# Edresson/VoiceSplit

Hardware: AMD Instinct MI355X
Metric: utterances/sec (3 s clips, B=64/GPU) fwd+bwd, channels-last bf16 activations / tape, bf16 MFMA, fp32 accumulate / statistics / master weights (higher is better)
Workload: dtype bf16 (conv activations and tape stored as bf16; bf16 MFMA operands in the convs, the LSTM / head contractions and the BPTT, f16 operands in the forward recurrence; fp32 accumulate, BatchNorm statistics, gate arithmetic / cell state, loss head, master weights)

## Files before the change

### include/voicesplit_hip.h

```cpp
#ifndef VOICESPLIT_HIP_H
#define VOICESPLIT_HIP_H

#include <stddef.h>
#include <stdint.h>

#ifdef __cplusplus
extern "C" {
#endif
#if defined(__GNUC__)
#pragma GCC visibility push(default)
#endif

#define VS_ABI_VERSION 11

#define VS_ACT_RELU 0
#define VS_ACT_MISH 1
#define VS_ACT_NONE 2
#define VS_ACT_SIGMOID 3

#define VS_MATH_FP32 0
#define VS_MATH_F16X3 1
#define VS_MATH_BF16 2

#define VS_BN_EVAL 0
// ... 227 lines not shown
  size_t total_bytes;
  size_t z[7];
  size_t a[7];
  size_t z8;
  size_t feat;
  size_t bn_scale, bn_shift, bn_mean, bn_invstd;
  size_t gates;
  size_t cstate;
  size_t lstm_out;
  size_t fc1_out;
  size_t dlogits;
  size_t dfc1;
  size_t dlstm_out;
  size_t dsum;
  size_t dfeat;
  size_t grad0, grad1;
  size_t dvbias, conv_packed[6], pack_tmp, lstm_packed, lstm_packed_t, lstm_state, lstm_bwd_state;
  size_t consts;
  size_t bn_stats, bn_coef, first_acc, colsum_tmp, partials;
  size_t conv_scales;
  size_t gemm_scales;
  size_t lstm_bf16;
  size_t det_turn;
  size_t conv_packed_t[6];
} vs_tape_layout;

int vs_tape_layout_query(const vs_dims* dims, vs_tape_layout* out);
size_t vs_tape_bytes(const vs_dims* dims);

int vs_forward_train(const vs_dims* dims, const vs_params* params, const float* x, const float* dvec,
                     int conv_act, int bn_mode, void* tape, size_t tape_bytes, float* mask, void* stream);

int vs_backward(const vs_dims* dims, const vs_params* params, const float* x, const float* dvec,
                int conv_act, int bn_mode, void* tape, size_t tape_bytes,
                const float* mask, const float* dmask, const vs_grads* grads, void* stream);

int vs_conv64_pack_dgrad(const float* w, float* packed, int KT, int KF, void* stream);
size_t vs_conv64_wgrad_partial_floats(int KT, int KF);
int vs_conv64_wgrad(const float* dz, const float* in, float* partials, float* dw,
                    int B, int T, int F, int KT, int KF, int dil, void* stream);
int vs_conv64_wgrad_f16x3(const float* dz, const float* in, float* partials, float* dw, float* scratch8,
                          int B, int T, int F, int KT, int KF, int dil, void* stream);
int vs_set_wgrad_kernel(int mode);
int vs_set_conv_kernel(int mode);
int vs_set_lstm_kernel(int mode);

enum vs_option {
  VS_OPT_FWD_PROLOGUE = 0,
  VS_OPT_HEAD_LEAF_SIDE = 1,
  VS_OPT_FEAT_ROWS = 2,
  VS_OPT_HEAD_BWD_GEMM = 3,
  VS_OPT_ABLATION = 4,
  VS_OPT_DETERMINISTIC = 5,
  VS_OPT_COUNT = 6
};
int vs_set_option(int option, int value);
int vs_get_option(int option);

int vs_lstm_status(const vs_dims* dims, const void* tape, size_t tape_bytes, const void* workspace, size_t workspace_bytes, void* stream);

int vs_set_backward_overlap(int on);
int vs_bn_act_bwd(const float* da, const float* z, float* dz, int C, long long R, int L, int act, int bn_mode,
                  const float* scale, const float* shift, const float* mean, const float* invstd,
                  float* dgamma, float* dbeta, float* dbias, double* stats, float* coef, void* stream);
int vs_bn_act_bwd_first(const float* da, const float* z, const float* x, float* xpad, int B, int T, int F, int act, int bn_mode,
                        const float* scale, const float* shift, const float* mean, const float* invstd,
                        float* dgamma, float* dbeta, float* dbias, float* dw, double* stats, float* coef, double* acc, void* stream);
int vs_conv_last_dgrad(const float* dz, const float* w, float* din, int B, int T, int F, void* stream);
int vs_conv_last_wgrad_blocks(void);
int vs_conv_last_wgrad(const float* dz, const float* in, float* partials , float* dw,
                       int B, int T, int F, void* stream);
int vs_conv_first_wgrad(const float* dz, const float* x, double* acc, float* dw, int B, int T, int F, void* stream);
int vs_gemm(int layout_a, int layout_w, const float* A, int lda, const float* W, int ldw, float* C, int ldc,
            int M, int N, int K, const float* bias, const float* gate, int ldg, int a_relu, int w_relu, int act,
            int accumulate, int w_shift, int w_group, int splits, float* partials, void* stream);
int vs_gemm_f16x3(int layout_a, int layout_w, const float* A, int lda, const float* W, int ldw, float* C, int ldc,
                  int M, int N, int K, const float* bias, const float* gate, int ldg, int a_relu, int w_relu, int act,
                  int accumulate, float* scratch8, void* stream);
int vs_bilstm_recurrent_train(const float* xg, const float* packed_whh, float* state, float* out,
                              float* gates_save, float* c_save, int B, int T, int H, void* stream);
size_t vs_lstm_packed_t_floats(int H);
size_t vs_lstm_bwd_state_floats(int B, int H);
int vs_lstm_pack_t(const float* w_hh_fwd, const float* w_hh_bwd, float* packed_t, int H, void* stream);
int vs_bilstm_recurrent_bwd(const float* packed_t, float* state, float* gates, const float* c_all,
                            const float* dout, int B, int T, int H, void* stream);
int vs_lstm_pack_t_math(const float* w_hh_fwd, const float* w_hh_bwd, float* packed_t, int H, int math, void* stream);
int vs_bilstm_recurrent_bwd_math(const float* packed_t, float* state, float* gates, const float* c_all,
                                 const float* dout, int B, int T, int H, int math, void* stream);
int vs_sigmoid_bwd(const float* dmask, const float* mask, float* dlogits, long long n, void* stream);
int vs_colsum(const float* x, int ld, int groups, int rows, int N, float* out, int ldo, void* stream);

typedef struct vs_loss_dims {
  int B, T, F;
  int n_fft, hop, win;
  float min_level_db;
  float ref_level_db;
} vs_loss_dims;

size_t vs_sisnr_workspace_bytes(const vs_loss_dims* dims);
int vs_sisnr_loss(const vs_loss_dims* dims, const float* mixed, const float* mask, const float* target,
                  const float* phase, const int* seq_len, void* workspace, size_t workspace_bytes,
                  float* loss, float* dmask, float* est_wav, void* stream);

int vs_powerlaw_loss(const float* mixed, const float* mask, const float* target, long long n, float power,
                     float complex_loss_ratio, double* scratch, float* loss, float* dmask, void* stream);

size_t vs_audio_workspace_bytes(const vs_loss_dims* dims);
// ... 170 lines not shown
```

### voicesplit_amd/_lib.py

```python
import ctypes
import os
from ctypes import POINTER, Structure, c_char_p, c_double, c_float, c_int, c_longlong, c_size_t, c_void_p

_HERE = os.path.dirname(os.path.abspath(__file__))
LIB_PATH = os.path.join(_HERE, "libvoicesplit_hip.so")

ACT_RELU, ACT_MISH, ACT_NONE, ACT_SIGMOID = 0, 1, 2, 3
BN_EVAL, BN_TRAIN = 0, 1
MATH_FP32, MATH_F16X3, MATH_BF16 = 0, 1, 2
PROF_SLOTS = 29
PROF_NAMES = ("cnn1", "cnn2", "cnn3", "cnn4", "cnn5", "cnn6", "cnn7", "cnn8", "lstm_gemm", "lstm_rec", "head",
              "fwd_bn", "bwd_head", "bwd_lstm_rec", "bwd_lstm_gemm", "bwd_bn",
              "wgrad_cnn2", "wgrad_cnn3", "wgrad_cnn4", "wgrad_cnn5", "wgrad_cnn6", "wgrad_cnn7",
              "dgrad_cnn2", "dgrad_cnn3", "dgrad_cnn4", "dgrad_cnn5", "dgrad_cnn6", "dgrad_cnn7", "bwd_edge")
ABI_VERSION = 11
CODEC_DB01, CODEC_DBNORM, CODEC_LOG = 0, 1, 2
PAD_REFLECT, PAD_ZERO = 0, 1


class VsDims(Structure):
    _fields_ = [(n, c_int) for n in ("B", "T", "F", "E", "H", "FC1", "FC2", "math")]


class VsConvLayer(Structure):
# ... 233 lines not shown
    "vs_split_workspace_bytes": (c_size_t, [c_longlong, c_int]),
    "vs_split_point": (c_int, [_P, c_longlong, _P, _P, _P, c_int, _P, _P, _P, c_int, _P, c_size_t, _P]),
    "vs_mix_sequence": (c_int, [_P, c_longlong, _P, c_longlong, _P, c_int, c_int, c_int, _P, _P, _P, _P, _P, _P, _P, _P]),
    "vs_resample_plan": (c_int, [c_int, c_int, POINTER(VsResampleDims)]),
    "vs_resample_out_len": (c_longlong, [POINTER(VsResampleDims), c_longlong]),
    "vs_resample_bank": (c_int, [POINTER(VsResampleDims), _P, _P]),
    "vs_resample": (c_int, [POINTER(VsResampleDims), _P, _P, c_longlong, c_longlong, c_longlong, c_longlong, _P, c_longlong, c_longlong,
                            c_longlong, c_int, _P]),
    "vs_resample_clips": (c_int, [POINTER(VsResampleDims), _P, _P, c_longlong, _P, c_longlong, _P, _P, c_int, _P]),
    "vs_loudness_plan": (c_int, [c_int, POINTER(VsLoudnessDims)]),
    "vs_loudness_workspace_bytes": (c_size_t, [POINTER(VsLoudnessDims), c_longlong, c_int]),
    "vs_loudness": (c_int, [POINTER(VsLoudnessDims), _P, c_longlong, _P, _P, c_int, _P, _P, _P, _P, _P, _P, _P, c_size_t, _P]),
    "vs_scale_clips": (c_int, [_P, c_longlong, _P, _P, _P, c_int, _P]),
    "vs_stoi_plan": (c_int, [POINTER(VsStoiDims)]),
    "vs_stoi_workspace_bytes": (c_size_t, [POINTER(VsStoiDims), c_longlong, c_int]),
    "vs_stoi": (c_int, [POINTER(VsStoiDims), _P, _P, c_longlong, _P, _P, c_int, c_int, _P, _P, _P, _P, _P, _P, c_size_t, _P]),
    "vs_rir_shoebox": (c_int, [_P, _P, c_int, c_int, _P, _P]),
    "vs_fir_rows": (c_int, [_P, c_longlong, _P, _P, _P, _P, c_int, c_int, _P, c_int, c_int, c_int, _P, _P, _P, _P]),
    "vs_row_energy": (c_int, [_P, c_int, c_int, _P, _P]),
    "vs_fir_spectra_bytes": (c_size_t, [c_int, c_int]),
    "vs_fir_spectra": (c_int, [_P, _P, _P, c_int, c_int, _P, c_size_t, _P]),
    "vs_fir_fft_workspace_bytes": (c_size_t, [c_int, c_int, c_int]),
    "vs_fir_rows_fft": (c_int, [_P, c_longlong, _P, _P, _P, c_int, c_int, _P, c_size_t, c_int, c_int, _P, c_size_t, _P, _P, _P]),
}

_lib = None


class VoiceSplitHipError(RuntimeError):
    pass


def load(path: str = None) -> ctypes.CDLL:
    global _lib
    if _lib is not None and path is None:
        return _lib
    path = path or LIB_PATH
    if not os.path.isfile(path):
        raise VoiceSplitHipError(
            f"{path} not found: build it with `python -c 'import __graft_entry__ as g; g.build()'` "
            f"or `make -C voicesplit_amd/csrc`. There is no PyTorch/CPU fallback for this path.")
    lib = ctypes.CDLL(path)
    for name, (restype, argtypes) in SIGNATURES.items():
        fn = getattr(lib, name)
        fn.restype = restype
        fn.argtypes = argtypes
    if lib.vs_abi_version() != ABI_VERSION:
        raise VoiceSplitHipError(f"{path}: ABI version {lib.vs_abi_version()} != {ABI_VERSION}; rebuild")
    _apply_env_options(lib)
    _lib = lib
    return lib


OPTIONS = {"FWD_PROLOGUE": 0, "HEAD_LEAF_SIDE": 1, "FEAT_ROWS": 2, "HEAD_BWD_GEMM": 3, "ABLATION": 4, "DETERMINISTIC": 5}
_ENV_OPTIONS = {
    "VOICESPLIT_FWD_PROLOGUE": ("FWD_PROLOGUE", int),
    "VOICESPLIT_HEAD_LEAF_SIDE": ("HEAD_LEAF_SIDE", int),
    "VOICESPLIT_FEAT_ROWS": ("FEAT_ROWS", int),
    "VOICESPLIT_HEAD_BWD_GEMM": ("HEAD_BWD_GEMM", int),
    "VOICESPLIT_ABLATION": ("ABLATION", int),
    "VOICESPLIT_DETERMINISTIC": ("DETERMINISTIC", int),
}


def _apply_env_options(lib):
    for var, (name, conv) in _ENV_OPTIONS.items():
        v = os.environ.get(var)
        if v is None or v == "":
            continue
        try:
            value = conv(v)
        except ValueError as err:
            raise VoiceSplitHipError(f"{var}={v}: not a value of this switch ({err})") from None
        if lib.vs_set_option(OPTIONS[name], value) != 0:
            msg = lib.vs_last_error()
            raise VoiceSplitHipError(f"{var}={v}: {msg.decode() if msg else 'rejected by vs_set_option'}")


def set_option(name: str, value: int):
    lib = load()
    prev = lib.vs_get_option(OPTIONS[name])
    check(lib.vs_set_option(OPTIONS[name], int(value)), f"vs_set_option({name})")
    return prev


def get_option(name: str) -> int:
    return load().vs_get_option(OPTIONS[name])


def check(rc: int, what: str):
    if rc != 0:
        msg = load().vs_last_error()
        raise VoiceSplitHipError(f"{what} failed (rc={rc}): {msg.decode() if msg else '?'}")
```

### voicesplit_amd/csrc/capi.hip

```cpp
#include <stdarg.h>
#include <stdlib.h>
#include <string.h>

#include "../../include/voicesplit_hip.h"
#include "vs_internal.h"

static thread_local char g_err[512] = "";

void vs_set_error(const char* fmt, ...) {
  va_list ap;
  va_start(ap, fmt);
  vsnprintf(g_err, sizeof(g_err), fmt, ap);
  va_end(ap);
}

int g_vs_options[VS_OPT_COUNT] = { 1,  1,  1,  1,  0,  0};
thread_local unsigned* g_vs_turn = nullptr;

namespace {
struct Prof {
  bool on = false;
  int max_calls = 0;
  int calls[VS_PROF_SLOTS] = {0};
  hipEvent_t* ev = nullptr;
} g_prof;

}

VsProfScope::VsProfScope(int slot, hipStream_t s_) : s(s_), idx(-1) {
  if (!g_prof.on || g_prof.calls[slot] >= g_prof.max_calls) return;
  idx = (g_prof.calls[slot]++ * VS_PROF_SLOTS + slot) * 2;
  (void)hipEventRecord(g_prof.ev[idx], s);
}
VsProfScope::~VsProfScope() { if (idx >= 0) (void)hipEventRecord(g_prof.ev[idx + 1], s); }

extern "C" {

int vs_abi_version(void) { return VS_ABI_VERSION; }

int vs_set_option(int option, int value) {
  VS_REQUIRE(option >= 0 && option < VS_OPT_COUNT, "vs_set_option: unknown option %d", option);
  bool ok = true;
  switch (option) {
    case VS_OPT_FWD_PROLOGUE: case VS_OPT_HEAD_LEAF_SIDE: case VS_OPT_FEAT_ROWS: case VS_OPT_HEAD_BWD_GEMM: case VS_OPT_DETERMINISTIC:
      ok = value == 0 || value == 1; break;
    default: ok = value >= 0; break;
  }
  VS_REQUIRE(ok, "vs_set_option: value %d is outside the range of option %d", value, option);
  g_vs_options[option] = value;
  return 0;
}

int vs_get_option(int option) { return (option >= 0 && option < VS_OPT_COUNT) ? g_vs_options[option] : -1; }

int vs_profile_begin(int max_calls) {
  VS_REQUIRE(!g_prof.on, "profile: already enabled");
  VS_REQUIRE(max_calls > 0 && max_calls <= 4096, "profile: max_calls=%d out of range", max_calls);
  max_calls *= 8;
  const int n = max_calls * VS_PROF_SLOTS * 2;
  g_prof.ev = new hipEvent_t[n];
  for (int i = 0; i < n; ++i) VS_CHECK_HIP(hipEventCreate(&g_prof.ev[i]));
  for (int i = 0; i < VS_PROF_SLOTS; ++i) g_prof.calls[i] = 0;
  g_prof.max_calls = max_calls;
  g_prof.on = true;
  return 0;
}

int vs_profile_end(float* ms_total, int* calls) {
  VS_REQUIRE(g_prof.on, "profile: not enabled");
  g_prof.on = false;
  int rc = 0;
  for (int slot = 0; slot < VS_PROF_SLOTS; ++slot) {
    double tot = 0;
    for (int c = 0; c < g_prof.calls[slot]; ++c) {
      const int idx = (c * VS_PROF_SLOTS + slot) * 2;
      float ms = 0.f;
      hipError_t e = hipEventSynchronize(g_prof.ev[idx + 1]);
      if (e == hipSuccess) e = hipEventElapsedTime(&ms, g_prof.ev[idx], g_prof.ev[idx + 1]);
      if (e != hipSuccess) { vs_set_error("profile: %s", hipGetErrorString(e)); rc = -2; }
      tot += ms;
    }
    if (ms_total) ms_total[slot] = (float)tot;
    if (calls) calls[slot] = g_prof.calls[slot];
  }
  const int n = g_prof.max_calls * VS_PROF_SLOTS * 2;
  for (int i = 0; i < n; ++i) (void)hipEventDestroy(g_prof.ev[i]);
  delete[] g_prof.ev;
  g_prof.ev = nullptr;
  g_prof.max_calls = 0;
  return rc;
}
const char* vs_last_error(void) { return g_err; }

int vs_bn_fold(const float* gamma, const float* beta, const float* mean, const float* var, const float* conv_bias,
               float eps, int C, float* scale, float* shift, void* stream) {
  return vs_bn_fold_impl(gamma, beta, mean, var, conv_bias, eps, C, scale, shift, (hipStream_t)stream);
}
// ... 347 lines not shown
```

### voicesplit_amd/csrc/loss.hip

```cpp
#include <math.h>

#include "../../include/voicesplit_hip.h"
#include "stft_common.h"

namespace {

__global__ __launch_bounds__(256)
void overlap_add_bwd_kernel(const float* __restrict__ dwav, const float* __restrict__ env, float* __restrict__ dframes, VsStftShape s,
                            unsigned* __restrict__ amax = nullptr) {
  const long long n = (long long)s.B * s.T * s.win;
  float mx = 0.f;
  for (long long i = (long long)blockIdx.x * 256 + threadIdx.x; i < n; i += (long long)gridDim.x * 256) {
    const long long m = i / s.win;
    const int j = (int)(i - m * s.win);
    const int b = (int)(m / s.T), t = (int)(m - (long long)b * s.T);
    const int sp = s.hop * t - s.lead + j;
    const float v = (sp >= 0 && sp < s.S) ? dwav[(size_t)b * s.S + sp] / env[sp] : 0.f;
    dframes[i] = v;
    mx = fmaxf(mx, fabsf(v));
  }
  vs_absmax_commit(mx, amax);
}

__global__ __launch_bounds__(256)
void sisnr_moments_kernel(const float* __restrict__ est, const float* __restrict__ src, const int* __restrict__ len,
                          double* __restrict__ mom , VsStftShape s) {
  const int b = blockIdx.y;
  const int L = len ? (len[b] < s.S ? (len[b] > 0 ? len[b] : 0) : s.S) : s.S;
  double a[6] = {0, 0, 0, 0, 0, 0};
  for (int i = blockIdx.x * 256 + threadIdx.x; i < s.S; i += gridDim.x * 256) {
    const double e = est[(size_t)b * s.S + i], r = src[(size_t)b * s.S + i];
    a[0] += r;
    if (i < L) { a[1] += e; a[2] += r; a[3] += e * r; a[4] += e * e; a[5] += r * r; }
  }
  __shared__ double red[4][6];
#pragma unroll
  for (int q = 0; q < 6; ++q) {
#pragma unroll
    for (int o = 32; o > 0; o >>= 1) a[q] += __shfl_down(a[q], o, 64);
  }
  if ((threadIdx.x & 63) == 0) {
#pragma unroll
    for (int q = 0; q < 6; ++q) red[threadIdx.x >> 6][q] = a[q];
  }
  __syncthreads();
  if (threadIdx.x < 6) atomicAdd(&mom[b * 8 + threadIdx.x], (red[0][threadIdx.x] + red[1][threadIdx.x]) + (red[2][threadIdx.x] + red[3][threadIdx.x]));
}

__global__ void sisnr_finalize_kernel(const double* __restrict__ mom, const int* __restrict__ len, float* __restrict__ coef ,
                                      float* __restrict__ loss, VsStftShape s) {
  __shared__ double acc[64];
  const int tid = threadIdx.x;
  double part = 0.0;
  const double eps = 1e-16;
  for (int b = tid; b < s.B; b += 64) {
    const double nlen = len ? (double)len[b] : (double)s.S;
    const int Lm_i = len ? (len[b] < s.S ? (len[b] > 0 ? len[b] : 0) : s.S) : s.S;
    const double Lm = Lm_i;
    const double* m = mom + b * 8;
    const double mu_s = m[0] / nlen, mu_e = m[1] / nlen;
    const double Sze = m[1] - Lm * mu_e, Szs = m[2] - Lm * mu_s;
    const double dot = m[3] - mu_s * m[1] - mu_e * m[2] + Lm * mu_e * mu_s;
    const double Z = m[5] - 2 * mu_s * m[2] + Lm * mu_s * mu_s;
    const double E = m[4] - 2 * mu_e * m[1] + Lm * mu_e * mu_e;
    const double es = Z + eps;
    const double P = dot * dot * Z / (es * es);
    const double c = (es + eps) / (es * es);
    const double N = E - c * dot * dot + eps;
    const double snr = P / N;
    part += 10.0 * log10(snr + eps);
    const double k = 10.0 / (log(10.0) * (snr + eps)) * (-1.0 / s.B);
    const double gs = k * (2 * dot * Z / (es * es) / N + P / (N * N) * 2 * c * dot);
    const double ge = k * (-P / (N * N) * 2);
    const double gsum = gs * Szs + ge * Sze;
    float* o = coef + b * 8;
    o[0] = (float)gs; o[1] = (float)ge; o[2] = (float)(gsum / nlen); o[3] = (float)mu_s; o[4] = (float)mu_e;
    o[5] = (float)Lm_i;
  }
  acc[tid] = part;
  __syncthreads();
  if (tid == 0) {
    double t = 0;
    for (int i = 0; i < 64; ++i) t += acc[i];
    *loss = (float)(20.0 - t / s.B);
  }
}

__global__ __launch_bounds__(256)
void sisnr_grad_kernel(const float* __restrict__ est, const float* __restrict__ src, const float* __restrict__ coef,
                       float* __restrict__ dwav, VsStftShape s) {
  const int b = blockIdx.y;
  const float gs = coef[b * 8], ge = coef[b * 8 + 1], g0 = coef[b * 8 + 2], mu_s = coef[b * 8 + 3], mu_e = coef[b * 8 + 4];
  const int L = (int)coef[b * 8 + 5];
  for (int i = blockIdx.x * 256 + threadIdx.x; i < s.S; i += gridDim.x * 256) {
    float g = 0.f;
    if (i < L) {
      const float zs = src[(size_t)b * s.S + i] - mu_s, ze = est[(size_t)b * s.S + i] - mu_e;
      g = fmaf(gs, zs, fmaf(ge, ze, -g0));
    }
    dwav[(size_t)b * s.S + i] = g;
  }
}

__global__ __launch_bounds__(256)
void reim_to_dmask_kernel(const float* __restrict__ mixed, const float* __restrict__ mask, const float* __restrict__ phase,
                          const float* __restrict__ dreim, float* __restrict__ dmask, VsStftShape s) {
  const long long n = (long long)s.B * s.T * s.F;
  for (long long i = (long long)blockIdx.x * 256 + threadIdx.x; i < n; i += (long long)gridDim.x * 256) {
    const long long m = i / s.F;
    const int f = (int)(i - m * s.F);
    const float x = mixed[i], v = x * mask[i];
    float g = 0.f;
    if (v >= 0.f && v <= 1.f) {
      const float db = (v - 1.f) * (-s.min_level_db) + s.ref_level_db;
      const float mag = expf(db * kLn10Over20);
      float sn, cs;
      sincosf(phase[i], &sn, &cs);
      const float d = dreim[m * s.ldk + f] * expf(cs) + dreim[m * s.ldk + s.F + f] * expf(sn);
      g = x * (-s.min_level_db) * kLn10Over20 * mag * d;
    }
    dmask[i] = g;
  }
}

__global__ __launch_bounds__(256)
void powerlaw_kernel(const float* __restrict__ mixed, const float* __restrict__ mask, const float* __restrict__ target,
                     long long n, float power, float ratio, double* __restrict__ sums, float* __restrict__ dmask) {
  constexpr float kEps = 1e-16f;
  const float inv_n = (float)(1.0 / (double)n);
  double a0 = 0.0, a1 = 0.0;
  for (long long i = (long long)blockIdx.x * 256 + threadIdx.x; i < n; i += (long long)gridDim.x * 256) {
    const float mx = mixed[i];
    const float o = mx * mask[i] + kEps;
    const float t = target[i] + kEps;
    const float po = powf(o, power), pt = powf(t, power);
    const float ds = fabsf(pt) - fabsf(po), dc = pt - po;
    a0 += (double)(ds * ds);
    a1 += (double)(dc * dc);
    if (dmask) {
      const float sgn = po > 0.f ? 1.f : (po < 0.f ? -1.f : 0.f);
      const float dpo = (-2.f * ds * sgn - 2.f * ratio * dc) * inv_n;
      dmask[i] = mx * (power * powf(o, power - 1.f)) * dpo;
    }
  }
#pragma unroll
  for (int off = 32; off > 0; off >>= 1) {
    a0 += __shfl_down(a0, off, 64);
    a1 += __shfl_down(a1, off, 64);
  }
  __shared__ double sh[8];
  const int lane = threadIdx.x & 63, w = threadIdx.x >> 6;
  if (lane == 0) { sh[2 * w] = a0; sh[2 * w + 1] = a1; }
  __syncthreads();
  if (threadIdx.x == 0) {
    atomicAdd(&sums[0], sh[0] + sh[2] + sh[4] + sh[6]);
    atomicAdd(&sums[1], sh[1] + sh[3] + sh[5] + sh[7]);
  }
}

__global__ void powerlaw_finalize_kernel(const double* __restrict__ sums, long long n, float ratio, float* __restrict__ loss) {
  *loss = (float)(sums[0] / (double)n + (double)ratio * (sums[1] / (double)n));
}

}

extern "C" {

size_t vs_sisnr_workspace_bytes(const vs_loss_dims* d) {
  VsStftShape s;
  return vs_stft_make_shape(d, &s) ? 0 : vs_stft_layout(s).total;
}

int vs_sisnr_loss(const vs_loss_dims* d, const float* mixed, const float* mask, const float* target, const float* phase,
                  const int* seq_len, void* ws, size_t ws_bytes, float* loss, float* dmask, float* est_wav, void* stream_) {
  hipStream_t stream = (hipStream_t)stream_;
  VsStftShape s;
  if (int rc = vs_stft_make_shape(d, &s)) return rc;
  const VsStftLayout L = vs_stft_layout(s);
  VS_REQUIRE(mixed && mask && target && phase && loss, "sisnr_loss: NULL argument");
  if (int rc = vs_stft_check_envelope(s)) return rc;
  VS_REQUIRE(ws && (reinterpret_cast<uintptr_t>(ws) & 255) == 0 && ws_bytes >= L.total, "sisnr_loss: workspace too small or misaligned (%zu < %zu)", ws_bytes, L.total);
  const int M = s.B * s.T;
  const long long nspec = (long long)M * s.F;
  float* basis = at<float>(ws, L.basis);
  float* env = at<float>(ws, L.env);
  const bool split = vs_stft_split(s);
  unsigned* amax = at<unsigned>(ws, L.amax);
  float* scales = at<float>(ws, L.scales);
  vs_istft_basis_launch(basis, s, scales + 6, stream);
  vs_istft_envelope_launch(env, s, stream);
  float* reim[2] = {at<float>(ws, L.reim_e), at<float>(ws, L.reim_t)};
  float* frames[2] = {at<float>(ws, L.frames_e), at<float>(ws, L.frames_t)};
  float* wav[2] = {at<float>(ws, L.wav_e), at<float>(ws, L.wav_t)};
  if (split) VS_CHECK_HIP(hipMemsetAsync(amax, 0, (size_t)3 * VS_AMAX_SLOTS * 4, stream));
  const unsigned cap = split ? 2048 : 16384;
  vs_spec_to_reim_launch(mixed, mask, phase, reim[0], s, split ? amax : nullptr, vs_grid_for(nspec, cap), stream);
  vs_spec_to_reim_launch(target, nullptr, phase, reim[1], s, split ? amax + VS_AMAX_SLOTS : nullptr, vs_grid_for(nspec, cap), stream);
  for (int q = 0; q < 2; ++q) {
    if (split) if (int rc = vs_scale_from_absmax_impl(amax + q * VS_AMAX_SLOTS, VS_AMAX_SLOTS, scales + 2 * q, stream)) return rc;
    if (int rc = vs_stft_contract(split, 0, reim[q], s.ldk, basis, s.ldk, frames[q], s.win, M, s.win, s.K, scales + 2 * q, scales + 6, stream)) return rc;
    vs_overlap_add_launch(frames[q], env, wav[q], s, stream);
  }
  if (est_wav) VS_CHECK_HIP(hipMemcpyAsync(est_wav, wav[0], (size_t)s.B * s.S * 4, hipMemcpyDeviceToDevice, stream));
  double* mom = at<double>(ws, L.mom);
  float* coef = at<float>(ws, L.coef);
  VS_CHECK_HIP(hipMemsetAsync(mom, 0, (size_t)s.B * 8 * 8, stream));
  const int gx = vs_opt(VS_OPT_DETERMINISTIC) ? 1 : (s.S + 256 * 16 - 1) / (256 * 16);
  hipLaunchKernelGGL(sisnr_moments_kernel, dim3(gx, s.B), dim3(256), 0, stream, wav[0], wav[1], seq_len, mom, s);
  hipLaunchKernelGGL(sisnr_finalize_kernel, dim3(1), dim3(64), 0, stream, mom, seq_len, coef, loss, s);
  if (dmask) {
    float* dwav = at<float>(ws, L.dwav);
    hipLaunchKernelGGL(sisnr_grad_kernel, dim3(gx, s.B), dim3(256), 0, stream, wav[0], wav[1], coef, dwav, s);
    float* dframes = frames[0];
    hipLaunchKernelGGL(overlap_add_bwd_kernel, dim3(vs_grid_for((long long)M * s.win, cap)), dim3(256), 0, stream, dwav, env, dframes, s,
                       split ? amax + 2 * VS_AMAX_SLOTS : nullptr);
    float* dreim = reim[0];
    if (split) if (int rc = vs_scale_from_absmax_impl(amax + 2 * VS_AMAX_SLOTS, VS_AMAX_SLOTS, scales + 4, stream)) return rc;
    if (int rc = vs_stft_contract(split, 1, dframes, s.win, basis, s.ldk, dreim, s.ldk, M, s.K, s.win, scales + 4, scales + 6, stream)) return rc;
    hipLaunchKernelGGL(reim_to_dmask_kernel, dim3(vs_grid_for(nspec, 16384)), dim3(256), 0, stream, mixed, mask, phase, dreim, dmask, s);
  }
  VS_LAUNCH_CHECK();
  return 0;
}

int vs_powerlaw_loss(const float* mixed, const float* mask, const float* target, long long n, float power,
                     float complex_loss_ratio, double* scratch, float* loss, float* dmask, void* stream_) {
  hipStream_t stream = (hipStream_t)stream_;
  VS_REQUIRE(mixed && mask && target && scratch && loss, "powerlaw_loss: NULL argument");
  VS_REQUIRE(n > 0, "powerlaw_loss: n=%lld", n);
  VS_CHECK_HIP(hipMemsetAsync(scratch, 0, 2 * sizeof(double), stream));
  hipLaunchKernelGGL(powerlaw_kernel, dim3(vs_grid_for(n)), dim3(256), 0, stream, mixed, mask, target, n, power, complex_loss_ratio, scratch, dmask);
  hipLaunchKernelGGL(powerlaw_finalize_kernel, dim3(1), dim3(1), 0, stream, scratch, n, complex_loss_ratio, loss);
  VS_LAUNCH_CHECK();
  return 0;
}

}
```

### voicesplit_amd/csrc/stft.hip

```cpp
#include <math.h>

#include "../../include/voicesplit_hip.h"
#include "stft_common.h"

namespace {

__global__ void istft_basis_kernel(float* __restrict__ basis, VsStftShape s, float* __restrict__ scale2 = nullptr) {
  const int idx = blockIdx.x * blockDim.x + threadIdx.x;
  if (idx == 0 && scale2) {
    int e = 0;
    (void)frexpf(2.0f / (float)s.n_fft, &e);
    scale2[0] = ldexpf(1.f, 10 - e);
    scale2[1] = ldexpf(1.f, e - 10);
  }
  if (idx >= s.win * s.ldk) return;
  const int j = idx / s.ldk, k = idx - j * s.ldk;
  float v = 0.f;
  if (k < s.K) {
    const int kk = k < s.F ? k : k - s.F;
    const int n = (s.n_fft - s.win) / 2 + j;
    const int r = (int)(((long long)kk * n) % s.n_fft);
    float sn, cs;
    sincospif(2.0f * (float)r / (float)s.n_fft, &sn, &cs);
    const float c = (kk == 0 || 2 * kk == s.n_fft) ? 1.0f : 2.0f;
    v = (k < s.F ? cs : -sn) * c / (float)s.n_fft * hann_w(j, s);
  }
  basis[idx] = v;
}

__global__ void istft_envelope_kernel(float* __restrict__ env, VsStftShape s) {
  const int sp = blockIdx.x * blockDim.x + threadIdx.x;
  if (sp >= s.S) return;
  const int off = s.lead;
  float e = 0.f;
  int t_hi = (sp + off) / s.hop;
  if (t_hi > s.T - 1) t_hi = s.T - 1;
  for (int t = t_hi; t >= 0; --t) {
    const int j = sp - s.hop * t + off;
    if (j >= s.win) break;
    const float w = hann_w(j, s);
    e = fmaf(w, w, e);
  }
  env[sp] = e;
}

__global__ __launch_bounds__(256)
void spec_to_reim_kernel(const float* __restrict__ a, const float* __restrict__ b, const float* __restrict__ phase,
                         float* __restrict__ reim, VsStftShape s, unsigned* __restrict__ amax = nullptr) {
  const long long n = (long long)s.B * s.T * s.F;
  float mx = 0.f;
  for (long long i = (long long)blockIdx.x * 256 + threadIdx.x; i < n; i += (long long)gridDim.x * 256) {
    const long long m = i / s.F;
    const int f = (int)(i - m * s.F);
    float v = a[i];
    if (b) v *= b[i];
    const float db = (fminf(fmaxf(v, 0.f), 1.f) - 1.f) * (-s.min_level_db) + s.ref_level_db;
    const float mag = expf(db * kLn10Over20);
    float sn, cs;
    sincosf(phase[i], &sn, &cs);
    const float re = s.true_phase ? mag * cs : mag * expf(cs), im = s.true_phase ? mag * sn : mag * expf(sn);
    reim[m * s.ldk + f] = re;
    reim[m * s.ldk + s.F + f] = im;
    if (f == 0) for (int c = s.K; c < s.ldk; ++c) reim[m * s.ldk + c] = 0.f;
    mx = fmaxf(mx, fmaxf(fabsf(re), fabsf(im)));
  }
  vs_absmax_commit(mx, amax);
}

template <bool ZERO>
__global__ __launch_bounds__(256)
void stft_frames_kernel(const float* __restrict__ wav, float* __restrict__ frames, VsStftShape s, unsigned* __restrict__ amax = nullptr) {
  const long long n = (long long)s.B * s.T * s.win;
  float mx = 0.f;
  for (long long i = (long long)blockIdx.x * 256 + threadIdx.x; i < n; i += (long long)gridDim.x * 256) {
    const long long m = i / s.win;
    const int j = (int)(i - m * s.win);
    const int b = (int)(m / s.T), t = (int)(m - (long long)b * s.T);
    int idx = s.hop * t - s.lead + j;
    float v;
    if constexpr (ZERO) {
      v = (idx < 0 || idx >= s.S) ? 0.f : hann_w(j, s) * wav[(size_t)b * s.S + idx];
    } else {
      if (idx < 0) idx = -idx;
      if (idx >= s.S) idx = 2 * (s.S - 1) - idx;
      v = hann_w(j, s) * wav[(size_t)b * s.S + idx];
    }
    frames[i] = v;
    mx = fmaxf(mx, fabsf(v));
  }
  vs_absmax_commit(mx, amax);
}

__global__ void stft_basis_kernel(float* __restrict__ basis, VsStftShape s, float* __restrict__ scale2 = nullptr) {
  const int idx = blockIdx.x * blockDim.x + threadIdx.x;
  if (idx == 0 && scale2) { scale2[0] = 512.f; scale2[1] = 1.f / 512.f; }
  if (idx >= s.K * s.win) return;
  const int k = idx / s.win, j = idx - k * s.win;
  const int kk = k < s.F ? k : k - s.F;
  const int n = (s.n_fft - s.win) / 2 + j;
  const int r = (int)(((long long)kk * n) % s.n_fft);
  float sn, cs;
  sincospif(2.0f * (float)r / (float)s.n_fft, &sn, &cs);
  basis[idx] = k < s.F ? cs : -sn;
}

__global__ __launch_bounds__(256)
void overlap_add_kernel(const float* __restrict__ frames, const float* __restrict__ env, float* __restrict__ wav, VsStftShape s) {
  const int sp = blockIdx.x * 256 + threadIdx.x;
  const int b = blockIdx.y;
  if (sp >= s.S) return;
  wav[(size_t)b * s.S + sp] = stft_gather(frames, b, sp, s) / env[sp];
}

// ... 113 lines not shown
```

### voicesplit_amd/csrc/stft_common.h

```cpp
#pragma once
#include "vs_internal.h"

constexpr float kLn10Over20 = 0.11512925464970229f;

struct VsStftShape {
  int B, T, F, n_fft, hop, win, S;
  int lead;
  int K, ldk;
  float min_level_db, ref_level_db;
  int periodic;
  int true_phase;
};

struct VsStftLayout { size_t basis, fbasis, env, reim_e, reim_t, frames_e, frames_t, wav_e, wav_t, dwav, mom, coef, amax, scales, total; };

__device__ __forceinline__ float hann_w(int j, const VsStftShape& s) {
  const int den = s.periodic ? s.win : s.win - 1;
  return den > 0 ? 0.5f - 0.5f * cospif(2.0f * (float)j / (float)den) : 1.0f;
}

__device__ __forceinline__ float stft_gather(const float* __restrict__ frames, int b, int sp, const VsStftShape& s) {
  int t_hi = (sp + s.lead) / s.hop;
  if (t_hi > s.T - 1) t_hi = s.T - 1;
  float acc = 0.f;
  for (int t = t_hi; t >= 0; --t) {
    const int j = sp - s.hop * t + s.lead;
    if (j >= s.win) break;
    acc += frames[((size_t)b * s.T + t) * s.win + j];
  }
  return acc;
}

inline unsigned vs_grid_for(long long n, unsigned cap = 2048) {
  const long long nb = (n + 255) / 256;
  return (unsigned)(nb < 1 ? 1 : (nb < (long long)cap ? nb : (long long)cap));
}

void vs_stft_fill_shape(const vs_loss_dims* d, int B, int T, int S, VsStftShape* s);
int vs_stft_make_shape(const vs_loss_dims* d, VsStftShape* s);
VsStftLayout vs_stft_layout(const VsStftShape& s);
int vs_stft_check_envelope(const VsStftShape& s);
inline bool vs_stft_split(const VsStftShape& s) { return (size_t)s.B * s.T * s.ldk * 4 < (1ull << 32) - 4096; }
int vs_stft_contract(bool split, int layout_w, const float* A, int lda, const float* W, int ldw, float* C, int ldc, int M, int N, int K,
                     const float* a_scale2, const float* w_scale2, hipStream_t);
void vs_istft_basis_launch(float* basis, const VsStftShape& s, float* scale2, hipStream_t);
void vs_istft_envelope_launch(float* env, const VsStftShape& s, hipStream_t);
void vs_stft_basis_launch(float* basis, const VsStftShape& s, float* scale2, hipStream_t);
void vs_stft_frames_launch(const float* wav, float* frames, const VsStftShape& s, unsigned* amax, unsigned grid, hipStream_t,
                           int zero_pad = 0 );
void vs_spec_to_reim_launch(const float* a, const float* b, const float* phase, float* reim, const VsStftShape& s, unsigned* amax, unsigned grid,
                            hipStream_t);
void vs_overlap_add_launch(const float* frames, const float* env, float* wav, const VsStftShape& s, hipStream_t);
```

Before: 1437.

## Replace dense iSTFT basis contraction in loss with shared-memory mixed-radix FFT

```diff
diff --git a/include/voicesplit_hip.h b/include/voicesplit_hip.h
--- a/include/voicesplit_hip.h
+++ b/include/voicesplit_hip.h
@@ -303,7 +303,8 @@
   VS_OPT_HEAD_BWD_GEMM = 3,
   VS_OPT_ABLATION = 4,
   VS_OPT_DETERMINISTIC = 5,
-  VS_OPT_COUNT = 6
+  VS_OPT_LOSS_FFT = 6,
+  VS_OPT_COUNT = 7
 };
 int vs_set_option(int option, int value);
 int vs_get_option(int option);
diff --git a/voicesplit_amd/_lib.py b/voicesplit_amd/_lib.py
--- a/voicesplit_amd/_lib.py
+++ b/voicesplit_amd/_lib.py
@@ -309,7 +309,7 @@
     return lib
 
 
-OPTIONS = {"FWD_PROLOGUE": 0, "HEAD_LEAF_SIDE": 1, "FEAT_ROWS": 2, "HEAD_BWD_GEMM": 3, "ABLATION": 4, "DETERMINISTIC": 5}
+OPTIONS = {"FWD_PROLOGUE": 0, "HEAD_LEAF_SIDE": 1, "FEAT_ROWS": 2, "HEAD_BWD_GEMM": 3, "ABLATION": 4, "DETERMINISTIC": 5, "LOSS_FFT": 6}
 _ENV_OPTIONS = {
     "VOICESPLIT_FWD_PROLOGUE": ("FWD_PROLOGUE", int),
     "VOICESPLIT_HEAD_LEAF_SIDE": ("HEAD_LEAF_SIDE", int),
@@ -317,6 +317,7 @@
     "VOICESPLIT_HEAD_BWD_GEMM": ("HEAD_BWD_GEMM", int),
     "VOICESPLIT_ABLATION": ("ABLATION", int),
     "VOICESPLIT_DETERMINISTIC": ("DETERMINISTIC", int),
+    "VOICESPLIT_LOSS_FFT": ("LOSS_FFT", int),
 }
 
 
diff --git a/voicesplit_amd/csrc/capi.hip b/voicesplit_amd/csrc/capi.hip
--- a/voicesplit_amd/csrc/capi.hip
+++ b/voicesplit_amd/csrc/capi.hip
@@ -14,7 +14,7 @@
   va_end(ap);
 }
 
-int g_vs_options[VS_OPT_COUNT] = { 1,  1,  1,  1,  0,  0};
+int g_vs_options[VS_OPT_COUNT] = { 1,  1,  1,  1,  0,  0,  1};
 thread_local unsigned* g_vs_turn = nullptr;
 
 namespace {
@@ -43,6 +43,7 @@
   bool ok = true;
   switch (option) {
     case VS_OPT_FWD_PROLOGUE: case VS_OPT_HEAD_LEAF_SIDE: case VS_OPT_FEAT_ROWS: case VS_OPT_HEAD_BWD_GEMM: case VS_OPT_DETERMINISTIC:
+    case VS_OPT_LOSS_FFT:
       ok = value == 0 || value == 1; break;
     default: ok = value >= 0; break;
   }
diff --git a/voicesplit_amd/csrc/loss.hip b/voicesplit_amd/csrc/loss.hip
--- a/voicesplit_amd/csrc/loss.hip
+++ b/voicesplit_amd/csrc/loss.hip
@@ -14,8 +14,7 @@
     const long long m = i / s.win;
     const int j = (int)(i - m * s.win);
     const int b = (int)(m / s.T), t = (int)(m - (long long)b * s.T);
-    const int sp = s.hop * t - s.lead + j;
-    const float v = (sp >= 0 && sp < s.S) ? dwav[(size_t)b * s.S + sp] / env[sp] : 0.f;
+    const float v = stft_gather_bwd(dwav, env, b, t, j, s);
     dframes[i] = v;
     mx = fmaxf(mx, fabsf(v));
   }
@@ -109,17 +108,7 @@
   for (long long i = (long long)blockIdx.x * 256 + threadIdx.x; i < n; i += (long long)gridDim.x * 256) {
     const long long m = i / s.F;
     const int f = (int)(i - m * s.F);
-    const float x = mixed[i], v = x * mask[i];
-    float g = 0.f;
-    if (v >= 0.f && v <= 1.f) {
-      const float db = (v - 1.f) * (-s.min_level_db) + s.ref_level_db;
-      const float mag = expf(db * kLn10Over20);
-      float sn, cs;
-      sincosf(phase[i], &sn, &cs);
-      const float d = dreim[m * s.ldk + f] * expf(cs) + dreim[m * s.ldk + s.F + f] * expf(sn);
-      g = x * (-s.min_level_db) * kLn10Over20 * mag * d;
-    }
-    dmask[i] = g;
+    dmask[i] = vs_dmask_entry(mixed[i], mask[i], phase[i], dreim[m * s.ldk + f], dreim[m * s.ldk + s.F + f], s);
   }
 }
 
@@ -184,22 +173,30 @@
   const long long nspec = (long long)M * s.F;
   float* basis = at<float>(ws, L.basis);
   float* env = at<float>(ws, L.env);
+  float* reim[2] = {at<float>(ws, L.reim_e), at<float>(ws, L.reim_t)};
+  float* frames[2] = {at<float>(ws, L.frames_e), at<float>(ws, L.frames_t)};
+  float* wav[2] = {at<float>(ws, L.wav_e), at<float>(ws, L.wav_t)};
+  const bool fft = vs_opt(VS_OPT_LOSS_FFT) != 0 && vs_stft_fft_supported(s);
   const bool split = vs_stft_split(s);
   unsigned* amax = at<unsigned>(ws, L.amax);
   float* scales = at<float>(ws, L.scales);
-  vs_istft_basis_launch(basis, s, scales + 6, stream);
+  float* twiddles = reim[0];
+  const unsigned cap = split ? 2048 : 16384;
   vs_istft_envelope_launch(env, s, stream);
-  float* reim[2] = {at<float>(ws, L.reim_e), at<float>(ws, L.reim_t)};
-  float* frames[2] = {at<float>(ws, L.frames_e), at<float>(ws, L.frames_t)};
-  float* wav[2] = {at<float>(ws, L.wav_e), at<float>(ws, L.wav_t)};
-  if (split) VS_CHECK_HIP(hipMemsetAsync(amax, 0, (size_t)3 * VS_AMAX_SLOTS * 4, stream));
-  const unsigned cap = split ? 2048 : 16384;
-  vs_spec_to_reim_launch(mixed, mask, phase, reim[0], s, split ? amax : nullptr, vs_grid_for(nspec, cap), stream);
-  vs_spec_to_reim_launch(target, nullptr, phase, reim[1], s, split ? amax + VS_AMAX_SLOTS : nullptr, vs_grid_for(nspec, cap), stream);
-  for (int q = 0; q < 2; ++q) {
-    if (split) if (int rc = vs_scale_from_absmax_impl(amax + q * VS_AMAX_SLOTS, VS_AMAX_SLOTS, scales + 2 * q, stream)) return rc;
-    if (int rc = vs_stft_contract(split, 0, reim[q], s.ldk, basis, s.ldk, frames[q], s.win, M, s.win, s.K, scales + 2 * q, scales + 6, stream)) return rc;
-    vs_overlap_add_launch(frames[q], env, wav[q], s, stream);
+  if (fft) {
+    if (int rc = vs_stft_fft_twiddles(twiddles, s, stream)) return rc;
+    if (int rc = vs_istft_fft_frames(mixed, mask, target, phase, twiddles, frames[0], frames[1], s, stream)) return rc;
+    for (int q = 0; q < 2; ++q) vs_overlap_add_launch(frames[q], env, wav[q], s, stream);
+  } else {
+    vs_istft_basis_launch(basis, s, scales + 6, stream);
+    if (split) VS_CHECK_HIP(hipMemsetAsync(amax, 0, (size_t)3 * VS_AMAX_SLOTS * 4, stream));
+    vs_spec_to_reim_launch(mixed, mask, phase, reim[0], s, split ? amax : nullptr, vs_grid_for(nspec, cap), stream);
+    vs_spec_to_reim_launch(target, nullptr, phase, reim[1], s, split ? amax + VS_AMAX_SLOTS : nullptr, vs_grid_for(nspec, cap), stream);
+    for (int q = 0; q < 2; ++q) {
+      if (split) if (int rc = vs_scale_from_absmax_impl(amax + q * VS_AMAX_SLOTS, VS_AMAX_SLOTS, scales + 2 * q, stream)) return rc;
+      if (int rc = vs_stft_contract(split, 0, reim[q], s.ldk, basis, s.ldk, frames[q], s.win, M, s.win, s.K, scales + 2 * q, scales + 6, stream)) return rc;
+      vs_overlap_add_launch(frames[q], env, wav[q], s, stream);
+    }
   }
   if (est_wav) VS_CHECK_HIP(hipMemcpyAsync(est_wav, wav[0], (size_t)s.B * s.S * 4, hipMemcpyDeviceToDevice, stream));
   double* mom = at<double>(ws, L.mom);
@@ -211,13 +208,17 @@
   if (dmask) {
     float* dwav = at<float>(ws, L.dwav);
     hipLaunchKernelGGL(sisnr_grad_kernel, dim3(gx, s.B), dim3(256), 0, stream, wav[0], wav[1], coef, dwav, s);
-    float* dframes = frames[0];
-    hipLaunchKernelGGL(overlap_add_bwd_kernel, dim3(vs_grid_for((long long)M * s.win, cap)), dim3(256), 0, stream, dwav, env, dframes, s,
-                       split ? amax + 2 * VS_AMAX_SLOTS : nullptr);
-    float* dreim = reim[0];
-    if (split) if (int rc = vs_scale_from_absmax_impl(amax + 2 * VS_AMAX_SLOTS, VS_AMAX_SLOTS, scales + 4, stream)) return rc;
-    if (int rc = vs_stft_contract(split, 1, dframes, s.win, basis, s.ldk, dreim, s.ldk, M, s.K, s.win, scales + 4, scales + 6, stream)) return rc;
-    hipLaunchKernelGGL(reim_to_dmask_kernel, dim3(vs_grid_for(nspec, 16384)), dim3(256), 0, stream, mixed, mask, phase, dreim, dmask, s);
+    if (fft) {
+      if (int rc = vs_istft_fft_dmask(dwav, env, mixed, mask, phase, twiddles, dmask, s, stream)) return rc;
+    } else {
+      float* dframes = frames[0];
+      hipLaunchKernelGGL(overlap_add_bwd_kernel, dim3(vs_grid_for((long long)M * s.win, cap)), dim3(256), 0, stream, dwav, env, dframes, s,
+                         split ? amax + 2 * VS_AMAX_SLOTS : nullptr);
+      float* dreim = reim[0];
+      if (split) if (int rc = vs_scale_from_absmax_impl(amax + 2 * VS_AMAX_SLOTS, VS_AMAX_SLOTS, scales + 4, stream)) return rc;
+      if (int rc = vs_stft_contract(split, 1, dframes, s.win, basis, s.ldk, dreim, s.ldk, M, s.K, s.win, scales + 4, scales + 6, stream)) return rc;
+      hipLaunchKernelGGL(reim_to_dmask_kernel, dim3(vs_grid_for(nspec, 16384)), dim3(256), 0, stream, mixed, mask, phase, dreim, dmask, s);
+    }
   }
   VS_LAUNCH_CHECK();
   return 0;
diff --git a/voicesplit_amd/csrc/stft.hip b/voicesplit_amd/csrc/stft.hip
--- a/voicesplit_amd/csrc/stft.hip
+++ b/voicesplit_amd/csrc/stft.hip
@@ -54,11 +54,10 @@
     const int f = (int)(i - m * s.F);
     float v = a[i];
     if (b) v *= b[i];
-    const float db = (fminf(fmaxf(v, 0.f), 1.f) - 1.f) * (-s.min_level_db) + s.ref_level_db;
-    const float mag = expf(db * kLn10Over20);
-    float sn, cs;
-    sincosf(phase[i], &sn, &cs);
-    const float re = s.true_phase ? mag * cs : mag * expf(cs), im = s.true_phase ? mag * sn : mag * expf(sn);
+    const float mag = vs_spec_mag(v, s);
+    float pr, pi;
+    vs_phase_factors(phase[i], s, &pr, &pi);
+    const float re = mag * pr, im = mag * pi;
     reim[m * s.ldk + f] = re;
     reim[m * s.ldk + s.F + f] = im;
     if (f == 0) for (int c = s.K; c < s.ldk; ++c) reim[m * s.ldk + c] = 0.f;
diff --git a/voicesplit_amd/csrc/stft_common.h b/voicesplit_amd/csrc/stft_common.h
--- a/voicesplit_amd/csrc/stft_common.h
+++ b/voicesplit_amd/csrc/stft_common.h
@@ -19,6 +19,31 @@
   return den > 0 ? 0.5f - 0.5f * cospif(2.0f * (float)j / (float)den) : 1.0f;
 }
 
+__device__ __forceinline__ float vs_spec_mag(float v, const VsStftShape& s) {
+  const float db = (fminf(fmaxf(v, 0.f), 1.f) - 1.f) * (-s.min_level_db) + s.ref_level_db;
+  return expf(db * kLn10Over20);
+}
+__device__ __forceinline__ void vs_phase_factors(float phase, const VsStftShape& s, float* pr, float* pi) {
+  float sn, cs;
+  sincosf(phase, &sn, &cs);
+  *pr = s.true_phase ? cs : expf(cs);
+  *pi = s.true_phase ? sn : expf(sn);
+}
+
+__device__ __forceinline__ float vs_dmask_entry(float x, float mask, float phase, float dre, float dim, const VsStftShape& s) {
+  const float v = x * mask;
+  float g = 0.f;
+  if (v >= 0.f && v <= 1.f) {
+    const float db = (v - 1.f) * (-s.min_level_db) + s.ref_level_db;
+    const float mag = expf(db * kLn10Over20);
+    float sn, cs;
+    sincosf(phase, &sn, &cs);
+    const float d = dre * expf(cs) + dim * expf(sn);
+    g = x * (-s.min_level_db) * kLn10Over20 * mag * d;
+  }
+  return g;
+}
+
 __device__ __forceinline__ float stft_gather(const float* __restrict__ frames, int b, int sp, const VsStftShape& s) {
   int t_hi = (sp + s.lead) / s.hop;
   if (t_hi > s.T - 1) t_hi = s.T - 1;
@@ -29,6 +54,12 @@
     acc += frames[((size_t)b * s.T + t) * s.win + j];
   }
   return acc;
+}
+
+__device__ __forceinline__ float stft_gather_bwd(const float* __restrict__ dwav, const float* __restrict__ env, int b, int t, int j,
+                                                 const VsStftShape& s) {
+  const int sp = s.hop * t - s.lead + j;
+  return (sp >= 0 && sp < s.S) ? dwav[(size_t)b * s.S + sp] / env[sp] : 0.f;
 }
 
 inline unsigned vs_grid_for(long long n, unsigned cap = 2048) {
@@ -51,3 +82,10 @@
 void vs_spec_to_reim_launch(const float* a, const float* b, const float* phase, float* reim, const VsStftShape& s, unsigned* amax, unsigned grid,
                             hipStream_t);
 void vs_overlap_add_launch(const float* frames, const float* env, float* wav, const VsStftShape& s, hipStream_t);
+
+bool vs_stft_fft_supported(const VsStftShape& s);
+int vs_stft_fft_twiddles(float* twiddles, const VsStftShape& s, hipStream_t);
+int vs_istft_fft_frames(const float* mixed, const float* mask, const float* target, const float* phase, const float* twiddles,
+                        float* frames_e, float* frames_t, const VsStftShape& s, hipStream_t);
+int vs_istft_fft_dmask(const float* dwav, const float* env, const float* mixed, const float* mask, const float* phase,
+                       const float* twiddles, float* dmask, const VsStftShape& s, hipStream_t);
diff --git a/voicesplit_amd/csrc/stft_fft.hip b/voicesplit_amd/csrc/stft_fft.hip
--- /dev/null
+++ b/voicesplit_amd/csrc/stft_fft.hip
@@ -0,0 +1,231 @@
+#include <math.h>
+
+#include "../../include/voicesplit_hip.h"
+#include "fir_fft_core.h"
+#include "stft_common.h"
+#include "stft_fft_plan.h"
+
+namespace {
+
+using vs_fft::cadd;
+using vs_fft::cf;
+using vs_fft::cmul;
+using vs_fft::csub;
+using vs_fft::dft4;
+
+constexpr int kThreads = 256;
+constexpr int kHalf = kThreads / VS_SFFT_GROUP;
+
+__device__ __forceinline__ void dft_r(cf (&v)[2]) {
+  const cf a = cadd(v[0], v[1]), b = csub(v[0], v[1]);
+  v[0] = a; v[1] = b;
+}
+__device__ __forceinline__ void dft_r(cf (&v)[4]) { dft4(v[0], v[1], v[2], v[3]); }
+__device__ __forceinline__ void dft_r(cf (&v)[3]) {
+  const float s = 0.86602540378443864676f;
+  const cf t = cadd(v[1], v[2]), d = csub(v[1], v[2]);
+  const cf m = {v[0].x - 0.5f * t.x, v[0].y - 0.5f * t.y};
+  const cf q = {s * d.y, -s * d.x};
+  v[0] = cadd(v[0], t);
+  v[1] = cadd(m, q);
+  v[2] = csub(m, q);
+}
+__device__ __forceinline__ void dft_r(cf (&v)[5]) {
+  const float c1 = 0.30901699437494742410f, c2 = -0.80901699437494742410f;
+  const float s1 = 0.95105651629515357212f, s2 = 0.58778525229247312917f;
+  const cf a1 = cadd(v[1], v[4]), a2 = cadd(v[2], v[3]), b1 = csub(v[1], v[4]), b2 = csub(v[2], v[3]);
+  const cf p1 = {v[0].x + c1 * a1.x + c2 * a2.x, v[0].y + c1 * a1.y + c2 * a2.y};
+  const cf p2 = {v[0].x + c2 * a1.x + c1 * a2.x, v[0].y + c2 * a1.y + c1 * a2.y};
+  const cf q1 = {s1 * b1.x + s2 * b2.x, s1 * b1.y + s2 * b2.y};
+  const cf q2 = {s2 * b1.x - s1 * b2.x, s2 * b1.y - s1 * b2.y};
+  v[0] = {v[0].x + a1.x + a2.x, v[0].y + a1.y + a2.y};
+  v[1] = {p1.x + q1.y, p1.y - q1.x};
+  v[4] = {p1.x - q1.y, p1.y + q1.x};
+  v[2] = {p2.x + q2.y, p2.y - q2.x};
+  v[3] = {p2.x - q2.y, p2.y + q2.x};
+}
+
+template <int R>
+__device__ __forceinline__ void sfft_pass(const cf* __restrict__ in, cf* __restrict__ out, const cf* __restrict__ tw, int n, int ns, int tstep,
+                                          int t) {
+  const int nb = n / R;
+  const float inv_ns = 1.0f / (float)ns;
+  for (int j = t; j < nb; j += kHalf) {
+    const int k = vs_sfft_k(j, ns, inv_ns);
+    cf v[R];
+#pragma unroll
+    for (int r = 0; r < R; ++r) v[r] = in[vs_sfft_src(j, r, nb)];
+    if (ns > 1) {
+#pragma unroll
+      for (int r = 1; r < R; ++r) v[r] = cmul(v[r], tw[vs_sfft_tw(k, r, tstep)]);
+    }
+    dft_r(v);
+#pragma unroll
+    for (int r = 0; r < R; ++r) out[vs_sfft_dst(j, k, r, R, ns)] = v[r];
+  }
+}
+
+__device__ __forceinline__ cf* sfft_run(const VsFftPlan& p, cf* a, cf* b, const cf* tw, int t) {
+  for (int i = 0; i < p.npass; ++i) {
+    const int ns = p.ns[i], ts = p.tstep[i];
+    switch (p.radix[i]) {
+      case 2: sfft_pass<2>(a, b, tw, p.n, ns, ts, t); break;
+      case 3: sfft_pass<3>(a, b, tw, p.n, ns, ts, t); break;
+      case 4: sfft_pass<4>(a, b, tw, p.n, ns, ts, t); break;
+      default: sfft_pass<5>(a, b, tw, p.n, ns, ts, t); break;
+    }
+    __syncthreads();
+    cf* c = a; a = b; b = c;
+  }
+  return a;
+}
+
+__global__ void sfft_twiddle_kernel(cf* __restrict__ tw, int n) {
+  const int i = blockIdx.x * blockDim.x + threadIdx.x;
+  if (i >= n) return;
+  float sn, cs;
+  sincospif(2.0f * (float)i / (float)n, &sn, &cs);
+  tw[i] = {cs, -sn};
+}
+
+__global__ __launch_bounds__(kThreads)
+void istft_fft_kernel(const float* __restrict__ mixed, const float* __restrict__ mask, const float* __restrict__ target,
+                      const float* __restrict__ phase, const cf* __restrict__ tw_g, float* __restrict__ frames_e,
+                      float* __restrict__ frames_t, VsStftShape s, VsFftPlan p, int ngroups) {
+  extern __shared__ float4 sfft_lds[];
+  cf* const sm = reinterpret_cast<cf*>(sfft_lds);
+  const int N = s.n_fft, tid = threadIdx.x, h = tid / kHalf, t = tid - h * kHalf;
+  const int M = s.B * s.T, n0 = (N - s.win) / 2;
+  const float inv_n = 1.0f / (float)N;
+  cf* const tw = sm;
+  cf* const est = sm + N;
+  cf* const tgt = sm + 3 * (size_t)N;
+  for (int i = tid; i < N; i += kThreads) tw[i] = tw_g[i];
+  for (int g = blockIdx.x; g < ngroups; g += gridDim.x) {
+    const int mA = 2 * g, mB = mA + 1;
+    for (int f = tid; f < s.F; f += kThreads) {
+      const size_t iA = (size_t)mA * s.F + f, iB = (size_t)mB * s.F + f;
+      float pr, pi;
+      vs_phase_factors(phase[iA], s, &pr, &pi);
+      const float mgA = vs_spec_mag(mixed[iA] * mask[iA], s), mtA = vs_spec_mag(target[iA], s);
+      const float eAr = mgA * pr, eAi = mgA * pi, tAr = mtA * pr, tAi = mtA * pi;
+      float eBr = 0.f, eBi = 0.f, tBr = 0.f, tBi = 0.f;
+      if (mB < M) {
+        vs_phase_factors(phase[iB], s, &pr, &pi);
+        const float mgB = vs_spec_mag(mixed[iB] * mask[iB], s), mtB = vs_spec_mag(target[iB], s);
+        eBr = mgB * pr; eBi = mgB * pi; tBr = mtB * pr; tBi = mtB * pi;
+      }
+      if (f == 0 || 2 * f == N) {
+        est[f] = {eBr, eAr};
+        tgt[f] = {tBr, tAr};
+      } else {
+        est[f] = {eAi + eBr, eAr - eBi};
+        est[N - f] = {eBr - eAi, eAr + eBi};
+        tgt[f] = {tAi + tBr, tAr - tBi};
+        tgt[N - f] = {tBr - tAi, tAr + tBi};
+      }
+    }
+    __syncthreads();
+    cf* const a = sm + N + 2 * (size_t)N * h;
+    const cf* const res = sfft_run(p, a, a + N, tw, t);
+    const int which = (int)(res - a);
+    const cf* const re = est + which;
+    const cf* const rt = tgt + which;
+    for (int j = tid; j < s.win; j += kThreads) {
+      const float w = hann_w(j, s) * inv_n;
+      const cf e = re[n0 + j], q = rt[n0 + j];
+      frames_e[(size_t)mA * s.win + j] = e.y * w;
+      frames_t[(size_t)mA * s.win + j] = q.y * w;
+      if (mB < M) {
+        frames_e[(size_t)mB * s.win + j] = e.x * w;
+        frames_t[(size_t)mB * s.win + j] = q.x * w;
+      }
+    }
+    __syncthreads();
+  }
+}
+
+__global__ __launch_bounds__(kThreads)
+void istft_fft_bwd_kernel(const float* __restrict__ dwav, const float* __restrict__ env, const float* __restrict__ mixed,
+                          const float* __restrict__ mask, const float* __restrict__ phase, const cf* __restrict__ tw_g,
+                          float* __restrict__ dmask, VsStftShape s, VsFftPlan p, int ngroups) {
+  extern __shared__ float4 sfft_lds[];
+  cf* const sm = reinterpret_cast<cf*>(sfft_lds);
+  const int N = s.n_fft, tid = threadIdx.x, h = tid / kHalf, t = tid - h * kHalf;
+  const int M = s.B * s.T, n0 = (N - s.win) / 2;
+  const float inv_n = 1.0f / (float)N;
+  cf* const tw = sm;
+  for (int i = tid; i < N; i += kThreads) tw[i] = tw_g[i];
+  for (int g = blockIdx.x; g < ngroups; g += gridDim.x) {
+    for (int i = tid; i < VS_SFFT_GROUP * N; i += kThreads) {
+      const int hh = i >= N ? 1 : 0, n = i - hh * N, j = n - n0;
+      cf u = {0.f, 0.f};
+      if (j >= 0 && j < s.win) {
+        const int mA = (VS_SFFT_GROUP * g + hh) * 2, mB = mA + 1;
+        const float w = hann_w(j, s) * inv_n;
+        if (mA < M) { const int b = mA / s.T; u.x = stft_gather_bwd(dwav, env, b, mA - b * s.T, j, s) * w; }
+        if (mB < M) { const int b = mB / s.T; u.y = stft_gather_bwd(dwav, env, b, mB - b * s.T, j, s) * w; }
+      }
+      sm[N + 2 * (size_t)N * hh + n] = u;
+    }
+    __syncthreads();
+    cf* const a = sm + N + 2 * (size_t)N * h;
+    const cf* const res = sfft_run(p, a, a + N, tw, t);
+    const int which = (int)(res - a);
+    for (int i = tid; i < VS_SFFT_GROUP * s.F; i += kThreads) {
+      const int hh = i >= s.F ? 1 : 0, f = i - hh * s.F;
+      const int mA = (VS_SFFT_GROUP * g + hh) * 2, mB = mA + 1;
+      if (mA >= M) continue;
+      const cf* const r = sm + N + 2 * (size_t)N * hh + which;
+      const cf zk = r[f], zm = r[f == 0 ? 0 : N - f];
+      const float c = (f == 0 || 2 * f == N) ? 0.5f : 1.0f;
+      const size_t iA = (size_t)mA * s.F + f;
+      dmask[iA] = vs_dmask_entry(mixed[iA], mask[iA], phase[iA], c * (zk.x + zm.x), c * (zk.y - zm.y), s);
+      if (mB < M) {
+        const size_t iB = (size_t)mB * s.F + f;
+        dmask[iB] = vs_dmask_entry(mixed[iB], mask[iB], phase[iB], c * (zk.y + zm.y), c * (zm.x - zk.x), s);
+      }
+    }
+    __syncthreads();
+  }
+}
+
+unsigned sfft_grid(int ngroups, int lds_bytes) {
+  int per_cu = (160 * 1024) / lds_bytes;
+  per_cu = per_cu < 1 ? 1 : (per_cu > 4 ? 4 : per_cu);
+  const int cap = 256 * per_cu;
+  return (unsigned)(ngroups < cap ? ngroups : cap);
+}
+
+}
+
+bool vs_stft_fft_supported(const VsStftShape& s) {
+  VsFftPlan p;
+  return vs_sfft_make_plan(s.n_fft, &p);
+}
+
+int vs_stft_fft_twiddles(float* twiddles, const VsStftShape& s, hipStream_t stream) {
+  VS_REQUIRE(twiddles != nullptr, "stft_fft: NULL twiddle table");
+  hipLaunchKernelGGL(sfft_twiddle_kernel, dim3((s.n_fft + 255) / 256), dim3(256), 0, stream, reinterpret_cast<cf*>(twiddles), s.n_fft);
+  return 0;
+}
+
+int vs_istft_fft_frames(const float* mixed, const float* mask, const float* target, const float* phase, const float* twiddles,
+                        float* frames_e, float* frames_t, const VsStftShape& s, hipStream_t stream) {
+  VsFftPlan p;
+  VS_REQUIRE(vs_sfft_make_plan(s.n_fft, &p), "stft_fft: n_fft=%d has no plan", s.n_fft);
+  const int M = s.B * s.T, ngroups = (M + 1) / 2, lds = vs_sfft_lds_bytes(s.n_fft);
+  hipLaunchKernelGGL(istft_fft_kernel, dim3(sfft_grid(ngroups, lds)), dim3(kThreads), lds, stream, mixed, mask, target, phase,
+                     reinterpret_cast<const cf*>(twiddles), frames_e, frames_t, s, p, ngroups);
+  return 0;
+}
+
+int vs_istft_fft_dmask(const float* dwav, const float* env, const float* mixed, const float* mask, const float* phase,
+                       const float* twiddles, float* dmask, const VsStftShape& s, hipStream_t stream) {
+  VsFftPlan p;
+  VS_REQUIRE(vs_sfft_make_plan(s.n_fft, &p), "stft_fft: n_fft=%d has no plan", s.n_fft);
+  const int M = s.B * s.T, ngroups = (M + 2 * VS_SFFT_GROUP - 1) / (2 * VS_SFFT_GROUP), lds = vs_sfft_lds_bytes(s.n_fft);
+  hipLaunchKernelGGL(istft_fft_bwd_kernel, dim3(sfft_grid(ngroups, lds)), dim3(kThreads), lds, stream, dwav, env, mixed, mask, phase,
+                     reinterpret_cast<const cf*>(twiddles), dmask, s, p, ngroups);
+  return 0;
+}
diff --git a/voicesplit_amd/csrc/stft_fft_plan.h b/voicesplit_amd/csrc/stft_fft_plan.h
--- /dev/null
+++ b/voicesplit_amd/csrc/stft_fft_plan.h
@@ -0,0 +1,48 @@
+#pragma once
+
+#if defined(__HIPCC__)
+#define VS_SFFT_HD __host__ __device__ inline __attribute__((always_inline))
+#else
+#define VS_SFFT_HD inline
+#endif
+
+constexpr int VS_SFFT_MAX_PASSES = 12;
+constexpr int VS_SFFT_GROUP = 2;
+constexpr int VS_SFFT_LDS_BYTES = 64 * 1024;
+
+struct VsFftPlan {
+  int n, npass;
+  int radix[VS_SFFT_MAX_PASSES], ns[VS_SFFT_MAX_PASSES], tstep[VS_SFFT_MAX_PASSES];
+};
+
+inline int vs_sfft_lds_bytes(int n) { return (2 * VS_SFFT_GROUP + 1) * n * 8; }
+
+constexpr int VS_SFFT_MIN_N = 256;
+
+inline bool vs_sfft_make_plan(int n, VsFftPlan* p) {
+  if (n < VS_SFFT_MIN_N || (n & 1) || vs_sfft_lds_bytes(n) > VS_SFFT_LDS_BYTES) return false;
+  int rest = n, np = 0, ns = 1;
+  const int order[4] = {4, 2, 3, 5};
+  for (int o = 0; o < 4; ++o) {
+    const int R = order[o];
+    while (rest % R == 0) {
+      if (np == VS_SFFT_MAX_PASSES) return false;
+      p->radix[np] = R;
+      p->ns[np] = ns;
+      p->tstep[np] = n / (ns * R);
+      ns *= R;
+      rest /= R;
+      ++np;
+    }
+  }
+  if (rest != 1) return false;
+  p->n = n;
+  p->npass = np;
+  for (int i = np; i < VS_SFFT_MAX_PASSES; ++i) { p->radix[i] = 0; p->ns[i] = 0; p->tstep[i] = 0; }
+  return true;
+}
+
+VS_SFFT_HD int vs_sfft_k(int j, int ns, float inv_ns) { return j - (int)(((float)j + 0.5f) * inv_ns) * ns; }
+VS_SFFT_HD int vs_sfft_src(int j, int r, int n_over_r) { return j + r * n_over_r; }
+VS_SFFT_HD int vs_sfft_dst(int j, int k, int r, int R, int ns) { return (j - k) * R + k + r * ns; }
+VS_SFFT_HD int vs_sfft_tw(int k, int r, int tstep) { return k * r * tstep; }
```

Result: no change. 1442 (median of 6 runs) (+0.3%).
